# nkkk98/MyGPURaytracer

Measured on AMD Instinct MI355X. Metric: Mrays/s, higher is better.
Workload: dtype f32; 1 GPU; cornellObj.txt 1920x1080 depth 8, AA on, material sort on, 1 spp/step (BASELINE configs[3] / C4); arith=0, clock_warmup_steps=1188, rccl_ranks=1, parallelism=1 GPU

## Files before the change

mygpuraytracer_amd/csrc/pt_engine.hip:

```cpp
#include <hip/hip_runtime.h>
#include <stdint.h>
#include <stdio.h>
#include <string.h>
#include <string>
#include <vector>
#include <algorithm>
#include <cmath>

#include "../../include/mi355x_pathtracer.h"
#include "pt_kernels.h"
#include "pt_scene.h"
#include "pt_denoise.h"

namespace {

thread_local std::string g_last_error;
int set_error(int code, const std::string &msg) { g_last_error = msg; return code; }

#define HIPCHECK(expr)                                                                                   \
    do {                                                                                                 \
        hipError_t e_ = (expr);                                                                          \
        if (e_ != hipSuccess)                                                                            \
            return set_error(PTX_ERR_HIP, std::string(#expr) + ": " + hipGetErrorString(e_));            \
    } while (0)
// ... 205 lines not shown
    hipEvent_t ev_start = nullptr, ev_stop = nullptr;
    bool timing_valid = false;
    ptx_options opt{};
    DCamera cam{};
    int traceDepth = 0;
    TileMap tm{};
    int nbins = 1, nmats = 0, ngeoms = 0, maxTiles = 0, grid = 0, grid_seg = 0, cap = 0, cus = 0;
    bool grid_forced = false;
    int dbg_mesh_wg_per_cu = 0;
    int dbg_extra_lds = 0;
    int dbg_total_wg_per_cu = 0, dbg_nsets = 0;
    DevBuf<DGeom> d_geoms; DevBuf<DMaterial> d_mats; DevBuf<float> d_faces; DevBuf<uint8_t> d_texels;
    float *d_image = nullptr; DevBuf<float> d_image_own;
    DevBuf<float> d_fbuf[3];
    DevBuf<int32_t> d_ibuf[3];
    PathSoA soa[3];
    DevBuf<int32_t> d_counts;
    DevBuf<int32_t> d_chunk;
    DevBuf<int32_t> d_cache_chunk;
    DevBuf<int32_t> d_cache_super;
    int cache_gx = 0;
    DevBuf<int32_t> d_totals;
    int32_t *d_super = nullptr;
    DevBuf<float> d_tri9, d_gtab, d_aabb, d_objcull;
    std::vector<float> h_aabb;
    std::vector<int32_t> h_geom_type, h_roots, h_depths, h_wroots, h_wneeds;
    DevBuf<uint32_t> d_tile_geoms; bool tile_geoms_valid = false;
    DevBuf<BvhQuad> d_bvh_nodes; DevBuf<float> d_bvh_tris; DevBuf<int32_t> d_bvh_root, d_bvh_depth;
    DevBuf<BvhWide4> d_bvh_wide; DevBuf<int32_t> d_bvh_wroot, d_bvh_wneed;
    DevBuf<float> d_fnorm, d_cnorm;
    DevBuf<float> d_ldsblob;
    bool no_fast = false;
    bool no_last = false;
    bool force_fast = false;
    DevBuf<unsigned long long> d_keys; DevBuf<uint32_t> d_items; DevBuf<int32_t> d_item_count;
    DevBuf<int32_t> d_tile_done;
    size_t seg_items = 0;
    int nsuper = 1;
    size_t totals_bytes = 0, seg_totals = 0, field_stride = 0, seg_part = 0;
    int kmax = 1;
    long long split_min_paths = 1LL << 20;
    int lanes = 1;
    hipStream_t lane_stream[MAX_LANES] = {};
    hipEvent_t ev_fork = nullptr, ev_join[MAX_LANES] = {}, ev_chain[MAX_LANES] = {};
    struct Ahead { int first = 0, count = 0, next = 0, unfolded = 0; bool use_cache = false, valid = false, timed = false;
                   unsigned long long dir_bins = ~0ull, ntab_bins = 0ull; };
    Ahead ahead[MAX_LANES];
    int ahead_cur = -1, ahead_nxt = -1;
    bool render_ahead = false;
    int last_ahead_lane = -1;
    hipEvent_t ev_ahead0[MAX_LANES] = {}, ev_ahead1[MAX_LANES] = {};
    bool aux_dirty[MAX_LANES] = {};
    unsigned long long cache_dir_bins = ~0ull, cache_ntab_bins = 0ull;
    int cache_idx16 = 0;
    DevBuf<uchar4> d_pbo;
    DevBuf<float> d_denoised;
    DevBuf<float> d_albedo;
    DevBuf<float4> d_gbuf, d_dn_tmp;
    DevBuf<float> d_dn_out;
    bool gbuf_valid = false, dn_done = false;
    std::vector<uint8_t> h_spec;
    DevBuf<uint8_t> d_spec;
    DevBuf<float> d_var;
    bool var_done = false;
    DevBuf<unsigned long long> d_stamps;
    DevBuf<float> d_part;
// ... 146 lines not shown
    const int nb = t->nbins;
    const int ntri_lds = t->split_mesh ? 0 : t->ntri_lds;
    const int triWords = t->tri_lds ? sceneTableWords(ntri_lds, t->nmats, t->ngeoms) : 0;
    const size_t lds_bounce = sizeof(int32_t) * (bounceLdsWords(triWords, nb) + (t->split_mesh ? QUEUE_WORDS : 0)) + (size_t)t->dbg_extra_lds;
    const bool cache_on = t->cache_active();
    const bool use_cache = cache_on && t->cache_valid && iter_first != 1;
    const bool fill_cache = cache_on && !use_cache;
    const bool batched = K > 1 || t->lanes > 1;
    const bool needs_albedo = t->d_albedo && iter_first == 1;
    const bool fast_unsplit = !t->split_mesh && !t->no_fast && batched && !t->uses_uv && t->opt.sort_by_material &&
                              !needs_albedo && t->cull == 1 && t->tri_lds && t->bump_bits == 0 && t->ntri_lds == t->ntri &&
                              !t->d_bvh_root;
    auto per_cu = [&](bool first_bounce, bool last_bounce = false) {
        if (fast_unsplit && !defer && last_bounce) { if (const char *e = getenv("PTX_DEBUG_WG_LAST")) return std::max(1, atoi(e)); }
        if (fast_unsplit && !defer) { if (const char *e = getenv(first_bounce ? "PTX_DEBUG_WG_FIRST" : "PTX_DEBUG_WG_LATER")) return std::max(1, atoi(e)); }
        if (fast_unsplit) return defer ? PT_FAST_WAVES - 2 : first_bounce ? 20 : PT_FAST_WAVES;
        return t->split_mesh ? 32 : 8;
    };
    auto gx_of = [&](bool first_bounce, bool last_bounce = false) {
        int grid = t->grid_forced ? t->grid : t->cus * per_cu(first_bounce, last_bounce);
        if (t->dbg_total_wg_per_cu > 0) grid = t->cus * t->dbg_total_wg_per_cu;
        int g = grid / K;
        if (!t->grid_forced && t->dbg_total_wg_per_cu <= 0) {
            const int base = t->cus * (fast_unsplit ? (defer ? PT_FAST_WAVES - 2 : PT_FAST_WAVES) : t->split_mesh ? 16 : 8) / K;
            g = std::min(g, std::max(base, t->maxTiles / 8));
        }
        if (g < 64 && t->dbg_total_wg_per_cu <= 0) g = 64;
        if (g > t->maxTiles) g = t->maxTiles;
        if (g > t->grid_seg) g = t->grid_seg;
        if (g > grid) g = grid;
        return g < 1 ? 1 : g;
    };
    const int gx_first = gx_of(true), gx_later = gx_of(false);
    const int gx_last = gx_of(false, true);
    const int grid = t->cus * (t->dbg_total_wg_per_cu > 0 ? t->dbg_total_wg_per_cu : per_cu(false));
    const int gx = gx_later;
    const int nsuper = (gx + 63) / 64;
    const size_t chunk_cap = (size_t)nb * t->grid_seg;
    const size_t seg_counts = (2 * (size_t)nb + 1) * t->maxTiles, seg_chunk = 2 * 3 * chunk_cap, seg_totals = t->seg_totals;
    int32_t *counts_all = t->d_counts + seg0 * seg_counts, *counts_scat = counts_all + (size_t)nb * t->maxTiles;
    auto chunks = [&](int bounce) { return t->d_chunk + seg0 * seg_chunk + (size_t)(bounce & 1) * 3 * chunk_cap; };
    auto totals = [&](int bounce, int which) { return t->d_totals + seg0 * seg_totals + ((size_t)bounce * 2 + which) * nb; };
    auto supers = [&](int bounce, int which) { return t->d_super + seg0 * seg_totals + ((size_t)bounce * 2 + which) * nb * t->nsuper; };
    if (t->aux_dirty[lane]) {
        HIPCHECK(hipMemsetAsync(t->d_totals + seg0 * seg_totals, 0, sizeof(int32_t) * seg_totals * (size_t)t->kmax, stream));
        if (t->d_part)
            HIPCHECK(hipMemset2DAsync(t->d_part + seg0 * t->seg_part + 3 * (size_t)t->cap, sizeof(float) * t->seg_part, 0,
                                      (size_t)t->cap / 8, (size_t)t->kmax, stream));
        t->aux_dirty[lane] = false;
    }

    auto kt_begin = [&](int kind) -> int {
        if (!t->ktiming) return PTX_OK;
        if (t->kev_used + 2 > t->kev.size()) {
            hipEvent_t a, b2;
            HIPCHECK(hipEventCreate(&a)); HIPCHECK(hipEventCreate(&b2));
            t->kev.push_back(a); t->kev.push_back(b2);
        }
        if (t->kev_kind.size() < t->kev.size() / 2) t->kev_kind.resize(t->kev.size() / 2);
        t->kev_kind[t->kev_used / 2] = kind;
        HIPCHECK(hipEventRecord(t->kev[t->kev_used], stream));
        return PTX_OK;
    };
    auto kt_end = [&]() -> int {
        if (!t->ktiming) return PTX_OK;
        HIPCHECK(hipEventRecord(t->kev[t->kev_used + 1], stream));
        t->kev_used += 2;
// ... 22 lines not shown
        for (int k = 0; k < 3; k++) if (bp.sc.cull && !(std::fabs(t->cam.position[k]) <= 0.5f * CULL_FAR_ORIGIN)) bp.sc.cull = 2;
        bp.sc.ldsblob = t->d_ldsblob;
        const bool from_cache = (b == 1 && cache_on), to_cache = (first && cache_on);
        bp.in = from_cache ? t->soa[2] : soa_shift(t->soa[b & 1], seg0 * t->cap);
        bp.stage = to_cache ? t->soa[2] : soa_shift(t->soa[1 - (b & 1)], seg0 * t->cap);
        bp.in_totals = first ? nullptr : from_cache ? t->d_cache_totals : totals(b - 1, 0);
        bp.in_super = first ? nullptr : from_cache ? t->d_cache_super : supers(b - 1, 0);
        bp.in_chunk = first ? nullptr : from_cache ? t->d_cache_chunk : chunks(b - 1);
        const int gx_b = first ? gx_first : gx_later;
        bp.in_gx = from_cache ? t->cache_gx : (b == 1 ? gx_first : gx_later);
        bp.seg_in_totals = from_cache ? 0 : seg_totals; bp.seg_in_chunk = from_cache ? 0 : seg_chunk;
        bp.image = t->d_image;
        bp.iter = iter_first; bp.iter_stride = stride; bp.traceDepth = t->traceDepth; bp.bounce = b;
        bp.aa = t->opt.antialiasing; bp.dof = t->opt.depth_of_field; bp.sort = t->opt.sort_by_material; bp.uses_uv = t->uses_uv; bp.dir_bins = batch_dir_bins;
        bp.ntab_bins = batch_ntab_bins; bp.apps = t->opt.apps_variant; bp.albedo = t->d_albedo;
        bp.in_dir_bins = from_cache ? t->cache_dir_bins : bp.dir_bins; bp.in_ntab_bins = from_cache ? t->cache_ntab_bins : bp.ntab_bins;
        auto idx16_of = [&](int gxw) { return (!getenv("PTX_DEBUG_NO_IDX16") && (t->maxTiles + gxw - 1) / std::max(gxw, 1) <= 128) ? 1 : 0; };
        bp.idx16 = idx16_of(first ? gx_first : gx_later);
        bp.in_idx16 = first ? 0 : from_cache ? t->cache_idx16 : idx16_of(b == 1 ? gx_first : gx_later);
        bp.nbins = nb; bp.maxTiles = t->maxTiles;
        bp.counts_all = counts_all; bp.counts_scat = counts_scat;
        bp.chunk = to_cache ? t->d_cache_chunk : chunks(b); bp.chunk_cap = (int32_t)chunk_cap;
        bp.super_all = supers(b, 0); bp.super_scat = supers(b, 1);
        bp.totals_all = totals(b, 0); bp.totals_scat = totals(b, 1);
        bp.nsuper = t->nsuper;
        bp.seg_in = from_cache ? 0 : (size_t)t->cap; bp.seg_stage = to_cache ? 0 : (size_t)t->cap;
        bp.seg_counts = seg_counts; bp.seg_chunk = to_cache ? 0 : seg_chunk; bp.seg_totals = seg_totals;
        bp.stamps = t->d_stamps;
        bp.seg_part = t->seg_part;
        bp.part = batched ? t->d_part + seg0 * bp.seg_part : nullptr;
        bp.emit_count = (first && fill_cache) ? t->d_emit_count : nullptr;
        bp.emit_pix = t->d_emit_pix; bp.emit_rgb = t->d_emit_rgb;
        bp.fenced = reinterpret_cast<unsigned long long *>(t->d_stats + 65); bp.fence_slots = t->fence_slots; bp.fence_slots_cap = (uint32_t)t->cap;
        bp.tile_geoms = (first && t->tile_geoms_valid) ? t->d_tile_geoms : nullptr;
        if (t->split_mesh) {
            bp.keys = t->d_keys + seg0 * (size_t)t->cap; bp.seg_keys = (size_t)t->cap;
            bp.items = t->d_items + seg0 * t->seg_items; bp.seg_items = t->seg_items;
            bp.item_count = t->d_item_count + 2 * seg0;
            bp.item_cursor = bp.item_count + K;
            bp.tile_done = (first && t->d_tile_done) ? t->d_tile_done + seg0 * (size_t)t->maxTiles : nullptr;
            HIPCHECK(hipMemsetAsync(bp.item_count, 0, sizeof(int32_t) * 2 * (size_t)K, stream));
            KT(first ? 0 : 1, { int rcl = launch_bounce(t, first, 1, needs_albedo, dim3(gx_b, K), lds_bounce, stream, bp); if (rcl != PTX_OK) return rcl; });
            const int mesh_gx = std::max(1, t->cus * (t->dbg_mesh_wg_per_cu > 0 ? t->dbg_mesh_wg_per_cu : PT_MESH_WG_PER_CU) / K);
            KT(2, { t->ks->mesh(first ? 1 : 0, dim3(mesh_gx, K), sizeof(int32_t) * ((size_t)t->bvh_stack * 256 + 32 * MESH_GEOM_WORDS), stream, &bp, t->bvh_stack);
                    t->ks->finish(first ? 1 : 0, dim3(std::max(1, grid / K), K), stream, &bp); });
            const size_t lds_pass2 = sizeof(int32_t) * ((size_t)ldsHeadWords(nb) + TILE);
            KT(3, { int rcl = launch_bounce(t, first, 2, needs_albedo, dim3(gx_b, K), lds_pass2, stream, bp); if (rcl != PTX_OK) return rcl; });
        } else {
            bp.keys = nullptr; bp.items = nullptr; bp.item_count = nullptr; bp.item_cursor = nullptr; bp.seg_keys = bp.seg_items = 0; bp.tile_done = nullptr;
            KT(first ? 0 : 1, { int rcl = launch_bounce(t, first, 0, needs_albedo, dim3(gx_b, K), lds_bounce, stream, bp, gx_last); if (rcl != PTX_OK) return rcl; });
        }

        if (first && fill_cache) {
            HIPCHECK(hipMemcpyAsync(t->d_cache_totals, totals(0, 0), sizeof(int32_t) * 2 * nb, hipMemcpyDeviceToDevice, stream));
            HIPCHECK(hipMemcpyAsync(t->d_cache_super, supers(0, 0), sizeof(int32_t) * 2 * nb * t->nsuper, hipMemcpyDeviceToDevice, stream));
            t->cache_gx = gx_b;
            t->cache_dir_bins = bp.dir_bins; t->cache_ntab_bins = bp.ntab_bins; t->cache_idx16 = bp.idx16;
            t->cache_valid = true;
        }
        if (t->capture_bounce == b && t->d_cap && b + 1 < t->traceDepth) {
            int32_t *gs = t->d_cap + 3 * (size_t)t->cap + nb, *ga = gs + chunk_cap + 1;
            hipLaunchKernelGGL(k_capture_prefix, dim3(1), dim3(64), 0, stream, bp.chunk, (int)chunk_cap, nb * gx_b, gs, ga);
            hipLaunchKernelGGL(k_capture, dim3(std::min(1024, (t->cap + 255) / 256)), dim3(256), 0, stream, bp.stage, bp.chunk, (int)chunk_cap,
                               nb * gx_b, gs, ga, t->cap, t->d_cap, t->d_cap_f, bp.idx16);
            HIPCHECK(hipMemcpyAsync(t->d_cap + 3 * (size_t)t->cap, totals(b, 1), sizeof(int32_t) * nb, hipMemcpyDeviceToDevice, stream));
            t->cap_filled = true;
// ... 189 lines not shown
    t->tm.tile_rows = opt.tile_world > 1 ? opt.tile_rows : H;
    fastdiv_magic((uint32_t)W, t->tm.w_mul, t->tm.w_sh);
    fastdiv_magic((uint32_t)t->tm.tile_rows, t->tm.rows_mul, t->tm.rows_sh);
    t->tm.owned = owned_pixels(W, H, t->tm.tile_rows, opt.tile_rank, opt.tile_world);
    t->maxTiles = (std::max(t->tm.owned, 1) + TILE - 1) / TILE;
    t->cap = t->maxTiles * TILE;
    t->nbins = opt.sort_by_material ? (nmaterials > 0 ? nmaterials : 1) : 1;
    {
        int per_cu = 16;
        if (const char *e = getenv("PTX_DEBUG_WG_PER_CU")) { per_cu = std::max(1, atoi(e)); t->grid_forced = true; }
        t->cus = prop.multiProcessorCount;
        t->grid = std::max(1, std::min(t->maxTiles, prop.multiProcessorCount * per_cu));
    }
    t->grid_seg = std::max(1, std::min(t->grid, t->maxTiles));
    t->nsuper = (t->grid_seg + 63) / 64;
    HostScene hs;
    SceneSwitches sw;
    sw.no_wide_bvh = getenv("PTX_DEBUG_NO_WIDE_BVH") != nullptr; sw.no_chunks = getenv("PTX_DEBUG_NO_CHUNKS") != nullptr;
    sw.no_dir_skip = getenv("PTX_DEBUG_NO_DIR_SKIP") != nullptr; sw.no_normal_codes = getenv("PTX_DEBUG_NO_NORMAL_CODES") != nullptr;
    sw.force_split = getenv("PTX_DEBUG_FORCE_SPLIT") != nullptr; sw.no_objcull = getenv("PTX_DEBUG_NO_OBJCULL") != nullptr;
    if (const int rc = pt_prepare_scene(ngeoms, geoms, nmaterials, materials, opt, t->tm.owned, t->nbins, prop.sharedMemPerBlock, sw, hs)) return fail(rc);
    static_cast<SceneFacts &>(*t) = hs;
    {
        size_t mem_free = 0, mem_total = 0;
        if (opt.batch <= 0 && hipMemGetInfo(&mem_free, &mem_total) != hipSuccess) { mem_free = mem_total = 0; (void)hipGetLastError(); }
        const char *e = getenv("PTX_DEBUG_MEM_BUDGET_MB");
        const LaunchPlan plan = plan_launch_sets(t->tm.owned, t->nbins, t->maxTiles, opt, kmax_cap, mem_free, mem_total, e ? std::max(1LL, atoll(e)) : 0);
        if (!plan.refusal.empty()) { set_error(PTX_ERR_UNSUPPORTED, plan.refusal); return fail(PTX_ERR_UNSUPPORTED); }
        t->kmax = *kmax_used = plan.kmax;
        t->lanes = plan.lanes;
    }
    t->no_fast = getenv("PTX_DEBUG_NO_FAST") != nullptr;
    t->no_last = getenv("PTX_DEBUG_NO_LAST") != nullptr;
    t->force_fast = getenv("PTX_DEBUG_FORCE_FAST") != nullptr;
    if (const char *e = getenv("PTX_DEBUG_TOTAL_WG_PER_CU")) t->dbg_total_wg_per_cu = std::max(0, atoi(e));
    if (const char *e = getenv("PTX_DEBUG_NSETS")) t->dbg_nsets = std::max(0, atoi(e));
    if (const char *e = getenv("PTX_DEBUG_EXTRA_LDS")) t->dbg_extra_lds = std::max(0, std::min(atoi(e), 32768)) & ~15;
    if (const char *e = getenv("PTX_DEBUG_MESH_WG_PER_CU")) t->dbg_mesh_wg_per_cu = std::max(0, atoi(e));
    if (const char *e = getenv("PTX_DEBUG_SPLIT_MIN")) t->split_min_paths = std::max(1LL, atoll(e));
    if (stream) { t->stream = (hipStream_t)stream; t->own_stream = false; }
    else {
        int prio_lo = 0, prio_hi = 0;
        if (hipDeviceGetStreamPriorityRange(&prio_lo, &prio_hi) != hipSuccess) { prio_lo = prio_hi = 0; (void)hipGetLastError(); }
        if (getenv("PTX_DEBUG_NO_PRIORITY")) prio_hi = prio_lo;
        HC(hipStreamCreateWithPriority(&t->stream, hipStreamNonBlocking, prio_hi));
        t->own_stream = true;
    }
    HC(hipEventCreate(&t->ev_start)); HC(hipEventCreate(&t->ev_stop));
    if (t->lanes > 1) {
        HC(hipEventCreateWithFlags(&t->ev_fork, hipEventDisableTiming));
        for (int l = 0; l < t->lanes; l++) {
            if (l) {
                int prio_lo = 0, prio = 0;
                if (hipDeviceGetStreamPriorityRange(&prio_lo, &prio) != hipSuccess || getenv("PTX_DEBUG_NO_PRIORITY")) { prio = 0; (void)hipGetLastError(); }
                if (const char *e = getenv("PTX_DEBUG_LANE_PRIO")) {
                    const char *q = e;
                    for (int k = 1; k <= l && q; k++) { prio = atoi(q); q = strchr(q, ','); if (q) q++; }
                }
                HC(hipStreamCreateWithPriority(&t->lane_stream[l], hipStreamNonBlocking, prio));
            }
            HC(hipEventCreateWithFlags(&t->ev_join[l], hipEventDisableTiming));
            HC(hipEventCreateWithFlags(&t->ev_chain[l], hipEventDisableTiming));
            if (l) { HC(hipEventCreate(&t->ev_ahead0[l])); HC(hipEventCreate(&t->ev_ahead1[l])); }
        }
    }
    HC(t->d_geoms.upload(hs.geoms)); HC(t->d_mats.upload(hs.mats)); HC(t->d_faces.upload(hs.faces)); HC(t->d_texels.upload(hs.texels));
// ... 861 lines not shown
```

mygpuraytracer_amd/csrc/pt_kernels.h:

```cpp
#pragma once
#include <hip/hip_runtime.h>
#include <stdint.h>

#include "pt_device.h"
#include "pt_bvh.h"

using namespace ptd;

namespace {

#ifndef PT_TILE
#define PT_TILE 256
#endif
#ifndef PT_MESH_WAVES
#define PT_MESH_WAVES 5
#endif
#ifndef PT_PARK_STATE
#define PT_PARK_STATE 1
#endif
#ifndef PT_FAST_WAVES
#define PT_FAST_WAVES 8
#endif
#ifndef PT_FAST_WAVES_FIRST
#define PT_FAST_WAVES_FIRST (PT_FAST_WAVES - 1)
#endif
#ifndef PT_FAST_WAVES_SPLIT
#define PT_FAST_WAVES_SPLIT 4
#endif
#ifndef PT_FAST_WAVES_SPLIT2
#define PT_FAST_WAVES_SPLIT2 5
#endif
#ifndef PT_BOUNCE_WAVES
#define PT_BOUNCE_WAVES 4
#endif
constexpr int TILE = PT_TILE;
constexpr int WAVES = TILE / 64;
constexpr int RANK_BITS = TILE <= 256 ? 8 : 9, BIN_BITS = 32 - 2 * RANK_BITS;
static_assert(TILE <= 512 && (TILE & (TILE - 1)) == 0, "tile size: a power of two up to 512 (9-bit ranks)");
#ifndef PT_WIN
#define PT_WIN 32
#endif
constexpr int WIN = PT_WIN, WIN_WORDS = 2 * (WIN + 1) + WIN + 2;
constexpr int ldsHeadWords(int nb) { return ((2 * WAVES * nb + 4 * nb + 1 + 8 + WIN_WORDS) + 3) & ~3; }
constexpr int REC_WORDS = 17 * TILE;
#ifndef PT_REC_ROWS_FAST0
#define PT_REC_ROWS_FAST0 16
#endif
constexpr int REC_ROWS_FAST0 = PT_REC_ROWS_FAST0;
static_assert(WIN <= 64 && (WIN & (WIN - 1)) == 0, "window of runs: one wave, binary search");
__host__ __device__ constexpr size_t bounceLdsWords(int tableWords, int nb) { return (size_t)tableWords + (size_t)ldsHeadWords(nb) + REC_WORDS; }
static_assert(ldsHeadWords(1) % 4 == 0 && ldsHeadWords(2) % 4 == 0 && ldsHeadWords(3) % 4 == 0 && ldsHeadWords(7) % 4 == 0 &&
// ... 102 lines not shown
struct TileMap {
    int32_t W, H, tile_rows, tile_rank, tile_world, owned;
    uint32_t w_mul, w_sh, rows_mul, rows_sh;
};

__device__ __forceinline__ int fastdiv(int n, uint32_t mul, uint32_t sh) {
    return sh == 255u ? n : (int)(__umulhi((uint32_t)n, mul) >> sh);
}

__device__ __forceinline__ void owned_pixel(const TileMap &tm, int i, int &x, int &y) {
    int r = fastdiv(i, tm.w_mul, tm.w_sh);
    x = i - r * tm.W;
    if (tm.tile_world <= 1) { y = r; return; }
    int k = fastdiv(r, tm.rows_mul, tm.rows_sh);
    y = (k * tm.tile_world + tm.tile_rank) * tm.tile_rows + (r - k * tm.tile_rows);
}

__device__ __forceinline__ int slot_to_pixel(const TileMap &tm, int slot) {
    if (tm.tile_world <= 1) return slot;
    int x, y;
    owned_pixel(tm, slot, x, y);
    return x + y * tm.W;
}

struct BounceParams {
    DScene sc;
    DCamera cam;
    TileMap tm;
    PathSoA in, stage;
    const int32_t *in_totals;
    const int32_t *in_super;
    const int32_t *in_chunk;
    int32_t in_gx;
    size_t seg_in_totals, seg_in_chunk;
    float *image;
    int32_t iter, traceDepth, bounce;
    int32_t iter_stride;
    unsigned long long *keys; uint32_t *items; int32_t *item_count;
    int32_t *item_cursor;
    size_t seg_keys, seg_items;
    const uint32_t *tile_geoms;
    int32_t *tile_done;
    int32_t aa, dof, sort;
    int32_t uses_uv;
    unsigned long long dir_bins;
    unsigned long long in_dir_bins, in_ntab_bins;
    int32_t idx16, in_idx16;
    unsigned long long ntab_bins;
    int32_t apps;
    float *albedo;
    int32_t nbins, maxTiles;
    int32_t *counts_all, *counts_scat;
    int32_t *chunk;
    int32_t chunk_cap;
    int32_t *super_all, *super_scat;
    int32_t *totals_all, *totals_scat;
    int32_t nsuper;
    size_t seg_in, seg_stage, seg_counts, seg_chunk, seg_totals, seg_part;
    unsigned long long *stamps;
    float *part;
    int32_t *emit_count; int32_t *emit_pix; float *emit_rgb;
    unsigned long long *fenced;
    uint32_t fence_slots;
    uint32_t fence_slots_cap;
};

// ... 79 lines not shown
```

mygpuraytracer_amd/csrc/pt_kernels.hip:

```cpp
#if PT_ARITH == 1
#define ptd ptd_arith1
#elif PT_ARITH == 2
#define ptd ptd_arith2
#elif defined(PT_ARITH) && PT_ARITH != 0
#error "PT_ARITH must be 0, 1 or 2"
#endif
#include <string.h>

#include "pt_kernels.h"

namespace {

__device__ __forceinline__ int32_t stage_key(int bin, int r_all, int r_scat) { return (int32_t)((uint32_t)bin | ((uint32_t)r_all << BIN_BITS) | ((uint32_t)r_scat << (BIN_BITS + RANK_BITS))); }
__device__ __forceinline__ void fence_report(const BounceParams &p) { atomicAdd(p.fenced, 1ull); }

__device__ __forceinline__ int sum_totals(const int32_t *t, int n) {
    int s = 0;
    for (int b = 0; b < n; b++) s += t[b];
    return s;
}

constexpr int ITEMS_PER_PASS = 4;
#ifdef PT_STAMPS
#define TI_STAMP(k) do { unsigned long long t1_ = __builtin_amdgcn_s_memtime(); st_acc[k] += t1_ - st_t0; st_t0 = t1_; } while (0)
#define TI_ARGS , unsigned long long *st_acc, unsigned long long &st_t0
#define TI_PASS , st_acc, st_t0
#else
#define TI_STAMP(k) do { } while (0)
#define TI_ARGS
#define TI_PASS
#endif
template <bool DEFER, bool PARK = false, bool SUBSET = false, bool DECODE = true>
__device__ __forceinline__ void tileIntersect(const DScene &sc, bool alive, Ray ray, bool need_uv, Hit &hit, int32_t *scratch,
                                              int32_t *tcnt, int &q, int tid, int lane, int wave, unsigned long long &key_out,
                                              uint32_t &mesh_out TI_ARGS, uint32_t subset = 0xffffffffu) {
    const float *gtab = reinterpret_cast<const float *>(pt_lds) + sc.ntri_lds * 24 + sc.nmats * 11;
    float *rayb = reinterpret_cast<float *>(scratch);
    unsigned long long *best = reinterpret_cast<unsigned long long *>(scratch + 6 * TILE);
    uint16_t *list = reinterpret_cast<uint16_t *>(scratch + 8 * TILE);
    uint16_t *listM = list + ITEMS_PER_PASS * TILE;
    constexpr int CAP = ITEMS_PER_PASS * TILE;
    uint32_t cube_mask = 0, sph_mask = 0, mesh_mask = 0;
    if (alive) {
        const uint32_t m = cullMask<SUBSET>(sc, ray, subset);
        cube_mask = m & sc.cube_bits; sph_mask = m & sc.sphere_bits; mesh_mask = m & sc.mesh_bits;
    }
    mesh_out = mesh_mask;
    if (DEFER) mesh_mask = 0;
    rayb[0 * TILE + tid] = ray.o.x; rayb[1 * TILE + tid] = ray.o.y; rayb[2 * TILE + tid] = ray.o.z;
    rayb[3 * TILE + tid] = ray.d.x; rayb[4 * TILE + tid] = ray.d.y; rayb[5 * TILE + tid] = ray.d.z;
    best[tid] = KEY_NONE;
    for (;;) {
        const int cc = (int)__popc(cube_mask), cs = (int)__popc(sph_mask), cm = (int)__popc(mesh_mask);
        const int nc = cc < ITEMS_PER_PASS ? cc : ITEMS_PER_PASS;
        const int ns = cs < ITEMS_PER_PASS - nc ? cs : ITEMS_PER_PASS - nc;
        const int nm = cm < ITEMS_PER_PASS - nc - ns ? cm : ITEMS_PER_PASS - nc - ns;
        int base[3], tot[3];
        const int cnt3[3] = {nc, ns, nm};
#pragma unroll
        for (int kind = 0; kind < 3; kind++) {
            const unsigned long long b0 = __ballot(cnt3[kind] & 1), b1 = __ballot(cnt3[kind] & 2), b2 = __ballot(cnt3[kind] & 4);
            base[kind] = wavePrefix(b0, lane) + 2 * wavePrefix(b1, lane) + 4 * wavePrefix(b2, lane);
            tot[kind] = __popcll(b0) + 2 * __popcll(b1) + 4 * __popcll(b2);
        }
        const unsigned long long left = __ballot(cc + cs + cm > nc + ns + nm);
        int wb0 = 0, wb1 = 0, wb2 = 0;
        if (lane == 0) {
            if (tot[0]) wb0 = atomicAdd(&tcnt[4 * q + 0], tot[0]);
            if (tot[1]) wb1 = atomicAdd(&tcnt[4 * q + 1], tot[1]);
            if (tot[2]) wb2 = atomicAdd(&tcnt[4 * q + 2], tot[2]);
            if (left) tcnt[4 * q + 3] = 1;
        }
        base[0] += __builtin_amdgcn_readfirstlane(wb0);
        base[1] += __builtin_amdgcn_readfirstlane(wb1);
        base[2] += __builtin_amdgcn_readfirstlane(wb2);
        for (int j = 0; j < nc; j++) {
            const int g = __ffs((int)cube_mask) - 1;
            cube_mask &= cube_mask - 1;
            list[base[0] + j] = (uint16_t)(tid | (g << RANK_BITS));
        }
        for (int j = 0; j < ns; j++) {
            const int g = __ffs((int)sph_mask) - 1;
            sph_mask &= sph_mask - 1;
            list[CAP - 1 - (base[1] + j)] = (uint16_t)(tid | (g << RANK_BITS));
        }
        for (int j = 0; j < nm; j++) {
            const int g = __ffs((int)mesh_mask) - 1;
            mesh_mask &= mesh_mask - 1;
            listM[base[2] + j] = (uint16_t)(tid | (g << RANK_BITS));
        }
        __syncthreads();
        const int totC = tcnt[4 * q + 0], totS = tcnt[4 * q + 1], totM = tcnt[4 * q + 2], more = tcnt[4 * q + 3];
        if (tid < 4) tcnt[4 * (q ^ 1) + tid] = 0;
        TI_STAMP(5);
#ifdef PT_STAMPS
        if (tid == 0) { st_acc[8] += totC + totS; st_acc[9] += totM; st_acc[10] += 1; }
#endif
        const int startS = (totC + 63) & ~63, startM = startS + ((totS + 63) & ~63);
// ... 147 lines not shown
template <bool FIRST, int MODE_, bool FAST = false>
__global__ __launch_bounds__(TILE, !FAST ? PT_BOUNCE_WAVES : MODE_ == 1 ? PT_FAST_WAVES_SPLIT : MODE_ == 2 ? PT_FAST_WAVES_SPLIT2 : FIRST ? PT_FAST_WAVES_FIRST : PT_FAST_WAVES) void k_bounce(const BounceParams p_in) {
    constexpr bool LAST = MODE_ == MODE_LAST;
    constexpr int MODE = LAST ? 0 : MODE_;
    static_assert(MODE_ >= 0 && MODE_ <= MODE_LAST && !(LAST && FIRST), "modes 0-2, and the light-only variant of a later unsplit bounce");
#ifdef PT_WGCLOCK
    const unsigned long long wg_t0 = wall_clock64();
#endif
    BounceParams p = p_in;
    if (FAST && MODE != 0) {
        p.sort = 1; p.albedo = nullptr; p.emit_count = nullptr; p.sc.cull = 1; p.sc.tri_lds = 1;
    }
    if (FAST && MODE == 0) {
        p.uses_uv = 0; p.sort = 1; p.albedo = nullptr; p.emit_count = nullptr; p.dof = 0;
        p.sc.cull = 1; p.sc.tri_lds = 2; p.sc.bump_bits = 0; p.sc.ntri_lds = p.sc.ntri; p.sc.bvh_root = nullptr;
    }
    const int tid = threadIdx.x, lane = tid & 63, wave = tid >> 6;
    const int nb = p.nbins;
    const int triWords = (MODE != 2 && p.sc.tri_lds) ? sceneLdsWords(p.sc) : 0;
    int32_t *lds = pt_lds + triWords;
    int32_t *w_all = lds, *w_scat = lds + WAVES * nb;
    int32_t *run_all = lds + 2 * WAVES * nb, *run_scat = run_all + nb;
    int32_t *tcs = run_scat + nb, *toff = tcs + nb;
    int32_t *tcnt = toff + nb + 1;
    int32_t *win = tcnt + 8;
    int tq = 0;
    int32_t *rec = lds + ldsHeadWords(nb);
    constexpr int R_PIX = (FAST && MODE == 0 ? REC_ROWS_FAST0 : 17) - 3, R_MG = R_PIX + 1, R_KEY = R_PIX + 2;
    uint32_t *qbuf = reinterpret_cast<uint32_t *>(rec + REC_WORDS);
    int32_t *qcnt = rec + REC_WORDS + QCAP, *qbase = qcnt + 1;
    if (MODE == 1 && tid == 0) *qcnt = 0;
    for (int k = tid; k < 2 * nb; k += TILE) run_all[k] = 0;
    if (tid < 8) tcnt[tid] = 0;
    __syncthreads();
    const int seg = blockIdx.y;
    const int iter = p.iter + seg * p.iter_stride;
    const PathSoA in_k = soa_offset(p.in, p.seg_in * seg), stage_k = soa_offset(p.stage, p.seg_stage * seg);
    int32_t *counts_all = p.counts_all + p.seg_counts * seg, *counts_scat = p.counts_scat + p.seg_counts * seg;
    int32_t *tile_np = counts_all + 2 * (size_t)nb * p.maxTiles;
    const bool direct = PT_DIRECT_STORE && MODE != 2 && (FAST || nb <= 64);
    int32_t *chunk_out = p.chunk + p.seg_chunk * seg;
    int32_t *super_all = p.super_all + p.seg_totals * seg, *super_scat = p.super_scat + p.seg_totals * seg;
    int32_t *totals_all = p.totals_all + p.seg_totals * seg, *totals_scat = p.totals_scat + p.seg_totals * seg;
    float *part = (FAST || p.part) ? p.part + p.seg_part * seg : nullptr;
    const bool batched = FAST || part != nullptr;
    const int32_t *in_totals = FIRST ? nullptr : p.in_totals + p.seg_in_totals * seg;
    const int32_t *in_chunk = FIRST ? nullptr : p.in_chunk + p.seg_in_chunk * seg;
    const int in_nruns = nb * p.in_gx;
    int v_tot = 0;
    if (!FIRST && nb <= 64 && lane < nb) v_tot = in_totals[nb + lane];
    const int n_in = FIRST ? p.tm.owned : nb <= 64 ? __builtin_amdgcn_readlane(waveInclusiveScan(v_tot, lane), 63) : sum_totals(in_totals + nb, nb);
    const int ntiles = (n_in + TILE - 1) / TILE;
    const int chunk = (ntiles + (int)gridDim.x - 1) / (int)gridDim.x;
    const int tile0 = min((int)blockIdx.x * chunk, ntiles), tile1 = min(tile0 + chunk, ntiles);
    auto binRanges = [&](unsigned long long mask, int &lo0, int &len0, int &lo1, int &len1) {
        int lo[2] = {0, 0}, hi[2] = {0, 0}, nr = 0, pos = 0;
        bool open = false;
        for (int b = 0; b < nb; b++) {
            const int tot = __builtin_amdgcn_readlane(v_tot, b);
            if (tot > 0) {
                const bool set = (mask >> b) & 1ull;
                if (set && !open) { if (nr < 2) lo[nr] = pos; open = true; }
                else if (!set && open) { if (nr < 2) hi[nr] = pos; nr++; open = false; }
            }
            pos += tot;
        }
// ... 76 lines not shown
    };
    auto fetch = [&](uint32_t li4, int idx_base, InRec &r, int jp) -> bool {
        const PathSoA in = soa_fresh(in_k);
        const uint32_t w = (uint32_t)ld_u(in.lsrc(), li4);
        uint32_t j;
        if (p.in_idx16) { j = (li4 >> 2) + (uint32_t)(int32_t)(int16_t)(w & 0xffffu); r.idx = idx_base + (int)(w >> 16); }
        else { j = w; r.idx = idx_base + ld_u(in.lidx(), li4); }
        if (__builtin_expect(j >= p.fence_slots, 0)) fence_report(p);
        const uint32_t j4 = min(j, p.fence_slots - 1u) << 2;
        const bool with_dir = (uint32_t)(jp - dir_lo0) < (uint32_t)dir_len0 || (uint32_t)(jp - dir_lo1) < (uint32_t)dir_len1;
        const bool coded_n = (uint32_t)(jp - ntab_lo0) < (uint32_t)ntab_len0 || (uint32_t)(jp - ntab_lo1) < (uint32_t)ntab_len1;
        typedef float quad __attribute__((ext_vector_type(4)));
        const uint32_t j16 = j4 << 2;
        const quad A = ld_u(reinterpret_cast<const quad *>(in.quadA()), j16), B = ld_u(reinterpret_cast<const quad *>(in.quadB()), j16);
        r.f[0] = A.x; r.f[1] = A.y; r.f[2] = A.z; r.pix = __float_as_int(A.w);
        r.f[6] = B.x; r.f[7] = B.y; r.f[8] = B.z; r.mg = __float_as_int(B.w);
        r.f[3] = r.f[4] = r.f[5] = 0.f; r.f[9] = r.f[10] = r.f[11] = 0.f; r.f[12] = r.f[13] = 0.f;
        if (with_dir) { const quad D = ld_u(reinterpret_cast<const quad *>(in.quadD()), j16); r.f[3] = D.x; r.f[4] = D.y; r.f[5] = D.z; if (p.uses_uv) r.f[13] = D.w; }
        if (!coded_n) { const quad C = ld_u(reinterpret_cast<const quad *>(in.quadC()), j16); r.f[9] = C.x; r.f[10] = C.y; r.f[11] = C.z; if (p.uses_uv) r.f[12] = C.w; }
        if (coded_n) {
            const int g = (int)min((uint32_t)(r.mg >> 16), (uint32_t)(p.sc.ngeoms - 1));
            const vec3 n = cubeNormalByCode(p.sc, reinterpret_cast<const float *>(pt_lds) + p.sc.ntri_lds * 24 + p.sc.nmats * 11, g, (r.pix >> 28) & 7);
            r.f[9] = n.x; r.f[10] = n.y; r.f[11] = n.z;
            r.pix &= 0x0fffffff;
        }
        if (__builtin_expect((uint32_t)r.pix >= (uint32_t)p.tm.owned, 0)) { fence_report(p); r.pix = 0; return false; }
        return true;
    };
    auto classifyRay = [&](const Hit &hit, const PathState &ps, int pix, int &bin, bool &pending) {
        classifyPath<FIRST>(p, iter, part, batched, hit, ps.color, pix, bin, pending);
    };
    int32_t *ccnt = qcnt + 2;
    int n_last = 0;
    int32_t k1_next = 0;
    if (MODE == 2) {
        for (int k = tid; k < 2 * WAVES * nb; k += TILE) lds[k] = 0;
        __syncthreads();
    }
    if (MODE == 2 && !FIRST && tile0 < tile1 && tile0 * TILE + tid < n_in) k1_next = ld_u(soa_fresh(stage_k).lsrc(), (uint32_t)(tile0 * TILE + tid) << 2);
    for (int tile = tile0; tile < tile1; tile++) {
#ifdef PT_STAMPS
        st_t0 = __builtin_amdgcn_s_memtime();
#endif
        const int i = tile * TILE + tid;
        bool alive = i < n_in;
        uint32_t tile_subset = 0xffffffffu;
        if (FIRST && MODE != 2 && p.tile_geoms) tile_subset = ((const __attribute__((address_space(4))) uint32_t *)p.tile_geoms)[tile];
        InRec cur;
        uint32_t li4 = 0;
        int idx_base = 0;
        if (!FIRST && MODE != 2) locate(tile, li4, idx_base);
        const PathSoA stage = soa_fresh(stage_k);
        PathState ps;
        int pix = 0;
        if (MODE != 2 && !direct && !LAST) for (int k = tid; k < 2 * WAVES * nb; k += TILE) lds[k] = 0;
        ps.o = ps.d = ps.color = V3(0.f, 0.f, 0.f);
        unsigned long long key = KEY_NONE;
        int32_t k1 = 0;
        if (MODE == 2 && !FIRST) {
            k1 = k1_next;
            if (tile + 1 < tile1 && i + TILE < n_in) k1_next = ld_u(soa_fresh(stage_k).lsrc(), (uint32_t)(i + TILE) << 2);
        }
        if (MODE == 2 && FIRST && p.tile_done && (p.tile_done + (size_t)p.maxTiles * seg)[tile]) {
            for (int b = tid; b < nb; b += TILE) {
                const int ca = counts_all[(size_t)b * p.maxTiles + tile], cs = counts_scat[(size_t)b * p.maxTiles + tile];
                counts_all[(size_t)b * p.maxTiles + tile] = run_all[b];
// ... 21 lines not shown
                owned_pixel(p.tm, i, x, y);
                pix = i;
                if (tile_subset != 0u) generateRay(p.cam, iter, p.traceDepth, p.aa != 0, p.dof != 0, x, y, ps);
            } else {
                const bool rec_ok = fetch(li4, idx_base, cur, min(i, n_in - 1));
                const vec3 intersect = V3(cur.f[0], cur.f[1], cur.f[2]);
                ps.d = V3(cur.f[3], cur.f[4], cur.f[5]);
                ps.color = V3(cur.f[6], cur.f[7], cur.f[8]);
                pix = cur.pix;
                Hit h;
                h.t = 1.f;
                h.n = V3(cur.f[9], cur.f[10], cur.f[11]);
                h.u = cur.f[12]; h.v = cur.f[13];
                const int mg = cur.mg;
                h.mat = mg & 0xffff; h.geom = mg >> 16;
                const int sidx = cur.idx;
#ifdef PT_STAMPS
                asm volatile("s_waitcnt vmcnt(0)" ::: "memory");
                STAMP(11);
#endif
                Rng rng; rng.seed(iter, sidx, 0);
                bool ended = (FAST && MODE == 0) ? scatterRay<false>(p.sc, ps, intersect, h, getMaterial(p.sc, h.mat), rng)
                                                 : scatterRay<true>(p.sc, ps, intersect, h, getMaterial(p.sc, h.mat), rng);
                if (ended && rec_ok) deposit(p.tm, p.image, part, batched, pix, ps.color, p.apps, p.fence_slots_cap);
                if (ended || !rec_ok) alive = false;
            }
        }
        STAMP(0);
        if (LAST) {
            n_last += __popcll(__ballot(alive));
            if (p.sc.light_bits == 0u) continue;
            Ray ray; ray.o = ps.o; ray.d = ps.d;
            const bool reach = alive && cullMask<true>(p.sc, ray, p.sc.light_bits) != 0u;
            Hit none;
            uint32_t mesh_cand = 0;
            tileIntersect<false, false, false, false>(p.sc, reach, ray, false, none, rec, tcnt, tq, tid, lane, wave, key, mesh_cand TI_PASS);
            if (reach && key != KEY_NONE) {
                const float *G = reinterpret_cast<const float *>(pt_lds) + p.sc.ntri_lds * 24 + p.sc.nmats * 11 + (int)((key >> 24) & 0xff) * GTAB_WORDS;
                Hit lh;
                lh.t = 1.f; lh.n = V3(0.f, 0.f, 0.f); lh.u = lh.v = 0.f; lh.geom = 0; lh.ncode = 0;
                lh.mat = __float_as_int(G[37]);
                int lbin = 0;
                bool lpend = false;
                classifyRay(lh, ps, pix, lbin, lpend);
            }
            STAMP(1);
            continue;
        }
        Hit hit;
        hit.t = -1.f; hit.n = V3(0.f, 0.f, 0.f); hit.u = hit.v = 0.f; hit.geom = 0; hit.mat = 0; hit.ncode = 0;
        if (FIRST && MODE == 0 && tile_subset == 0u) {
            int mbin = 0;
            bool mpend = false;
            if (alive) classifyRay(hit, ps, pix, mbin, mpend);
            if (tid == 0) tile_np[tile] = 0;
            if (tid == 0) run_all[p.sort ? p.sc.nmats - 1 : 0] += min(TILE, n_in - tile * TILE);
            continue;
        }
        if (FIRST && MODE == 1 && tile_subset == 0u && p.tile_done) {
            int mbin = 0;
            bool mpend = false;
            if (alive) classifyRay(hit, ps, pix, mbin, mpend);
            if (tid == 0) tile_np[tile] = 0;
            const int missbin = p.sort ? p.sc.nmats - 1 : 0, nalive = min(TILE, n_in - tile * TILE);
            for (int b = tid; b < nb; b += TILE) {
                counts_all[(size_t)b * p.maxTiles + tile] = b == missbin ? nalive : 0;
                counts_scat[(size_t)b * p.maxTiles + tile] = 0;
            }
            if (tid == 0) (p.tile_done + (size_t)p.maxTiles * seg)[tile] = 1;
            continue;
        }
        {
            Ray ray; ray.o = ps.o; ray.d = ps.d;
            uint32_t mesh_cand = 0;
            if (MODE == 1) {
                if (FIRST && tile_subset == 0u) __syncthreads();
                else tileIntersect<true, false, FIRST>(p.sc, alive, ray, p.uses_uv != 0, hit, rec, tcnt, tq, tid, lane, wave, key, mesh_cand TI_PASS, tile_subset);
// ... 58 lines not shown
            else {
                if (alive) intersectScene(p.sc, ray, hit);
                __syncthreads();
            }
        }
        STAMP(1);
    classify:
        if (MODE != 2 && direct && lane < nb) { w_all[wave * nb + lane] = 0; w_scat[wave * nb + lane] = 0; }
        if (MODE != 2 && alive) classifyRay(hit, ps, pix, bin, pending);
        STAMP(2);
        int r_all = 0, r_scat = 0;
        {
            const int abin = alive ? bin : -1, pbin = pending ? bin : -1;
            if (PT_RANK_SLICED && MODE != 2 && !FIRST && nb <= 16) {
                const unsigned long long A = __builtin_amdgcn_uicmp((uint32_t)abin, 0xffffffffu, 33), P = __builtin_amdgcn_uicmp((uint32_t)pbin, 0xffffffffu, 33);
                uint32_t slo = 0xffffffffu, shi = 0xffffffffu;
#pragma unroll
                for (int k = 0; k < 4; k++) {
                    if (k && (nb - 1) >> k == 0) break;
                    const unsigned long long Bk = __builtin_amdgcn_uicmp((uint32_t)bin & (1u << k), 0u, 33);
                    const bool set = (bin >> k) & 1;
                    slo &= set ? (uint32_t)Bk : ~(uint32_t)Bk;
                    shi &= set ? (uint32_t)(Bk >> 32) : ~(uint32_t)(Bk >> 32);
                }
                const uint32_t alo = slo & (uint32_t)A, ahi = shi & (uint32_t)(A >> 32), plo = slo & (uint32_t)P, phi = shi & (uint32_t)(P >> 32);
                const int ra = (int)__builtin_amdgcn_mbcnt_hi(ahi, __builtin_amdgcn_mbcnt_lo(alo, 0u));
                const int rs = (int)__builtin_amdgcn_mbcnt_hi(phi, __builtin_amdgcn_mbcnt_lo(plo, 0u));
                if (alive) {
                    r_all = ra; r_scat = rs;
                    if (ra == 0) {
                        w_all[wave * nb + bin] = __popc(alo) + __popc(ahi);
                        w_scat[wave * nb + bin] = __popc(plo) + __popc(phi);
                    }
                }
            } else {
                unsigned long long remaining = __builtin_amdgcn_uicmp((uint32_t)abin, 0xffffffffu, 33);
                while (remaining) {
                    int leader = __ffsll((long long)remaining) - 1;
                    int b = __builtin_amdgcn_readlane(abin, leader);
                    const unsigned long long m_all = __builtin_amdgcn_uicmp((uint32_t)abin, (uint32_t)b, 32), m_scat = __builtin_amdgcn_uicmp((uint32_t)pbin, (uint32_t)b, 32);
                    const int ra = wavePrefix(m_all, lane), rs = wavePrefix(m_scat, lane);
                    if (abin == b) { r_all = ra; r_scat = rs; }
                    if (lane == leader) {
                        w_all[wave * nb + b] = __popcll(m_all);
                        w_scat[wave * nb + b] = __popcll(m_scat);
                    }
                    remaining &= ~m_all;
                }
            }
        }
        STAMP(12);
        __syncthreads();
        STAMP(13);
        if (alive) {
            for (int w = 0; w < wave; w++) { r_all += w_all[w * nb + bin]; r_scat += w_scat[w * nb + bin]; }
        }
        int toff_bin = 0, npend_r = 0;
        if (direct) {
            int ln = lane;
            asm volatile("" : "+v"(ln));
            int ca = 0, cs = 0;
            if (ln < nb) for (int w = 0; w < WAVES; w++) { ca += w_all[w * nb + ln]; cs += w_scat[w * nb + ln]; }
            if (wave == 0 && ln < nb) {
                counts_all[(size_t)ln * p.maxTiles + tile] = MODE == 1 ? ca : run_all[ln];
                counts_scat[(size_t)ln * p.maxTiles + tile] = MODE == 1 ? cs : run_scat[ln];
                run_all[ln] += ca;
// ... 619 lines not shown
```

Before: 43140 Mrays/s.

## Compact last-bounce light rays into LDS pool and add wave-uniform fast paths

In the last-bounce light-reach pass, rays that can reach a light are compacted into a shared LDS pool across tiles and intersected only once a full tile's worth has accumulated. This cuts the number of idle lanes during light intersection. The change also adds a wave-uniform fast path for slot allocation in tileIntersect and for binning in the classify step. The packed-scan slot allocation replaces the three-ballot prefix computation. These changes add extra syncthreads and reuse the rec scratch buffer for the pool, which risks LDS aliasing with tileIntersect's own use of that scratch.

```diff
diff --git a/mygpuraytracer_amd/csrc/pt_engine.hip b/mygpuraytracer_amd/csrc/pt_engine.hip
--- a/mygpuraytracer_amd/csrc/pt_engine.hip
+++ b/mygpuraytracer_amd/csrc/pt_engine.hip
@@ -261,6 +261,7 @@
     DevBuf<float> d_ldsblob;
     bool no_fast = false;
     bool no_last = false;
+    bool last_inplace = false;
     bool force_fast = false;
     DevBuf<unsigned long long> d_keys; DevBuf<uint32_t> d_items; DevBuf<int32_t> d_item_count;
     DevBuf<int32_t> d_tile_done;
@@ -473,7 +474,8 @@
         return g < 1 ? 1 : g;
     };
     const int gx_first = gx_of(true), gx_later = gx_of(false);
-    const int gx_last = gx_of(false, true);
+    int gx_last = gx_of(false, true);
+    if (const char *e = getenv("PTX_DEBUG_GX_LAST")) gx_last = std::max(1, std::min(atoi(e), gx_last));
     const int grid = t->cus * (t->dbg_total_wg_per_cu > 0 ? t->dbg_total_wg_per_cu : per_cu(false));
     const int gx = gx_later;
     const int nsuper = (gx + 63) / 64;
@@ -562,6 +564,7 @@
         bp.emit_count = (first && fill_cache) ? t->d_emit_count : nullptr;
         bp.emit_pix = t->d_emit_pix; bp.emit_rgb = t->d_emit_rgb;
         bp.fenced = reinterpret_cast<unsigned long long *>(t->d_stats + 65); bp.fence_slots = t->fence_slots; bp.fence_slots_cap = (uint32_t)t->cap;
+        bp.last_inplace = t->last_inplace ? 1 : 0;
         bp.tile_geoms = (first && t->tile_geoms_valid) ? t->d_tile_geoms : nullptr;
         if (t->split_mesh) {
             bp.keys = t->d_keys + seg0 * (size_t)t->cap; bp.seg_keys = (size_t)t->cap;
@@ -817,6 +820,7 @@
     }
     t->no_fast = getenv("PTX_DEBUG_NO_FAST") != nullptr;
     t->no_last = getenv("PTX_DEBUG_NO_LAST") != nullptr;
+    t->last_inplace = getenv("PTX_DEBUG_LAST_INPLACE") != nullptr;
     t->force_fast = getenv("PTX_DEBUG_FORCE_FAST") != nullptr;
     if (const char *e = getenv("PTX_DEBUG_TOTAL_WG_PER_CU")) t->dbg_total_wg_per_cu = std::max(0, atoi(e));
     if (const char *e = getenv("PTX_DEBUG_NSETS")) t->dbg_nsets = std::max(0, atoi(e));
diff --git a/mygpuraytracer_amd/csrc/pt_kernels.h b/mygpuraytracer_amd/csrc/pt_kernels.h
--- a/mygpuraytracer_amd/csrc/pt_kernels.h
+++ b/mygpuraytracer_amd/csrc/pt_kernels.h
@@ -17,6 +17,12 @@
 #endif
 #ifndef PT_PARK_STATE
 #define PT_PARK_STATE 1
+#endif
+#ifndef PT_PACKED_SLOTS
+#define PT_PACKED_SLOTS 1
+#endif
+#ifndef PT_WAVE_UNIFORM
+#define PT_WAVE_UNIFORM 1
 #endif
 #ifndef PT_FAST_WAVES
 #define PT_FAST_WAVES 8
@@ -185,6 +191,7 @@
     const int32_t *in_super;
     const int32_t *in_chunk;
     int32_t in_gx;
+    int32_t last_inplace;
     size_t seg_in_totals, seg_in_chunk;
     float *image;
     int32_t iter, traceDepth, bounce;
diff --git a/mygpuraytracer_amd/csrc/pt_kernels.hip b/mygpuraytracer_amd/csrc/pt_kernels.hip
--- a/mygpuraytracer_amd/csrc/pt_kernels.hip
+++ b/mygpuraytracer_amd/csrc/pt_kernels.hip
@@ -30,6 +30,7 @@
 #define TI_ARGS
 #define TI_PASS
 #endif
+__device__ __forceinline__ int waveInclusiveScan(int v, int lane);
 template <bool DEFER, bool PARK = false, bool SUBSET = false, bool DECODE = true>
 __device__ __forceinline__ void tileIntersect(const DScene &sc, bool alive, Ray ray, bool need_uv, Hit &hit, int32_t *scratch,
                                               int32_t *tcnt, int &q, int tid, int lane, int wave, unsigned long long &key_out,
@@ -40,13 +41,18 @@
     uint16_t *list = reinterpret_cast<uint16_t *>(scratch + 8 * TILE);
     uint16_t *listM = list + ITEMS_PER_PASS * TILE;
     constexpr int CAP = ITEMS_PER_PASS * TILE;
-    uint32_t cube_mask = 0, sph_mask = 0, mesh_mask = 0;
+    uint32_t cube_mask = 0, sph_mask = 0, mesh_mask = 0, m_all = 0;
     if (alive) {
-        const uint32_t m = cullMask<SUBSET>(sc, ray, subset);
-        cube_mask = m & sc.cube_bits; sph_mask = m & sc.sphere_bits; mesh_mask = m & sc.mesh_bits;
+        m_all = cullMask<SUBSET>(sc, ray, subset);
+        cube_mask = m_all & sc.cube_bits; sph_mask = m_all & sc.sphere_bits; mesh_mask = m_all & sc.mesh_bits;
     }
     mesh_out = mesh_mask;
     if (DEFER) mesh_mask = 0;
+    bool uniform_wave = false;
+    if (SUBSET && PT_WAVE_UNIFORM) {
+        const uint32_t m0 = (uint32_t)__builtin_amdgcn_readfirstlane((int)m_all);
+        uniform_wave = __ballot(alive && m_all == m0) == ~0ull && __popc(m0 & (DEFER ? ~sc.mesh_bits : 0xffffffffu)) <= ITEMS_PER_PASS;
+    }
     rayb[0 * TILE + tid] = ray.o.x; rayb[1 * TILE + tid] = ray.o.y; rayb[2 * TILE + tid] = ray.o.z;
     rayb[3 * TILE + tid] = ray.d.x; rayb[4 * TILE + tid] = ray.d.y; rayb[5 * TILE + tid] = ray.d.z;
     best[tid] = KEY_NONE;
@@ -56,14 +62,29 @@
         const int ns = cs < ITEMS_PER_PASS - nc ? cs : ITEMS_PER_PASS - nc;
         const int nm = cm < ITEMS_PER_PASS - nc - ns ? cm : ITEMS_PER_PASS - nc - ns;
         int base[3], tot[3];
-        const int cnt3[3] = {nc, ns, nm};
+        unsigned long long left = 0ull;
+        if (SUBSET && PT_WAVE_UNIFORM && uniform_wave) {
+            const int u0 = __builtin_amdgcn_readfirstlane(nc), u1 = __builtin_amdgcn_readfirstlane(ns), u2 = __builtin_amdgcn_readfirstlane(nm);
+            base[0] = lane * u0; base[1] = lane * u1; base[2] = lane * u2;
+            tot[0] = 64 * u0; tot[1] = 64 * u1; tot[2] = 64 * u2;
+        } else {
+#if PT_PACKED_SLOTS
+            const int packed = nc | (ns << 10) | (nm << 20);
+            const int inc = waveInclusiveScan(packed, lane), exc = inc - packed;
+            const int all = __builtin_amdgcn_readlane(inc, 63);
+            base[0] = exc & 1023; base[1] = (exc >> 10) & 1023; base[2] = exc >> 20;
+            tot[0] = all & 1023; tot[1] = (all >> 10) & 1023; tot[2] = all >> 20;
+#else
+            const int cnt3[3] = {nc, ns, nm};
 #pragma unroll
-        for (int kind = 0; kind < 3; kind++) {
-            const unsigned long long b0 = __ballot(cnt3[kind] & 1), b1 = __ballot(cnt3[kind] & 2), b2 = __ballot(cnt3[kind] & 4);
-            base[kind] = wavePrefix(b0, lane) + 2 * wavePrefix(b1, lane) + 4 * wavePrefix(b2, lane);
-            tot[kind] = __popcll(b0) + 2 * __popcll(b1) + 4 * __popcll(b2);
-        }
-        const unsigned long long left = __ballot(cc + cs + cm > nc + ns + nm);
+            for (int kind = 0; kind < 3; kind++) {
+                const unsigned long long b0 = __ballot(cnt3[kind] & 1), b1 = __ballot(cnt3[kind] & 2), b2 = __ballot(cnt3[kind] & 4);
+                base[kind] = wavePrefix(b0, lane) + 2 * wavePrefix(b1, lane) + 4 * wavePrefix(b2, lane);
+                tot[kind] = __popcll(b0) + 2 * __popcll(b1) + 4 * __popcll(b2);
+            }
+#endif
+            left = __ballot(cc + cs + cm > nc + ns + nm);
+        }
         int wb0 = 0, wb1 = 0, wb2 = 0;
         if (lane == 0) {
             if (tot[0]) wb0 = atomicAdd(&tcnt[4 * q + 0], tot[0]);
@@ -277,6 +298,7 @@
     if (MODE == 1 && tid == 0) *qcnt = 0;
     for (int k = tid; k < 2 * nb; k += TILE) run_all[k] = 0;
     if (tid < 8) tcnt[tid] = 0;
+    if (LAST && tid == 0) tcs[0] = 0;
     __syncthreads();
     const int seg = blockIdx.y;
     const int iter = p.iter + seg * p.iter_stride;
@@ -419,6 +441,7 @@
     };
     int32_t *ccnt = qcnt + 2;
     int n_last = 0;
+    int32_t *pool_n = tcs;
     int32_t k1_next = 0;
     if (MODE == 2) {
         for (int k = tid; k < 2 * WAVES * nb; k += TILE) lds[k] = 0;
@@ -506,17 +529,51 @@
             if (p.sc.light_bits == 0u) continue;
             Ray ray; ray.o = ps.o; ray.d = ps.d;
             const bool reach = alive && cullMask<true>(p.sc, ray, p.sc.light_bits) != 0u;
-            Hit none;
-            uint32_t mesh_cand = 0;
-            tileIntersect<false, false, false, false>(p.sc, reach, ray, false, none, rec, tcnt, tq, tid, lane, wave, key, mesh_cand TI_PASS);
-            if (reach && key != KEY_NONE) {
-                const float *G = reinterpret_cast<const float *>(pt_lds) + p.sc.ntri_lds * 24 + p.sc.nmats * 11 + (int)((key >> 24) & 0xff) * GTAB_WORDS;
-                Hit lh;
-                lh.t = 1.f; lh.n = V3(0.f, 0.f, 0.f); lh.u = lh.v = 0.f; lh.geom = 0; lh.ncode = 0;
-                lh.mat = __float_as_int(G[37]);
-                int lbin = 0;
-                bool lpend = false;
-                classifyRay(lh, ps, pix, lbin, lpend);
+            const bool inplace = !FAST || p.last_inplace != 0;
+            const unsigned long long rb = __ballot(reach);
+            int pbase = 0;
+            if (!inplace && lane == 0 && rb) pbase = atomicAdd(pool_n, __popcll(rb));
+            int slot = inplace ? tid : __builtin_amdgcn_readfirstlane(pbase) + wavePrefix(rb, lane);
+            float *poolf = reinterpret_cast<float *>(rec);
+            auto pool_put = [&](int s) {
+                poolf[0 * TILE + s] = ray.o.x; poolf[1 * TILE + s] = ray.o.y; poolf[2 * TILE + s] = ray.o.z;
+                poolf[3 * TILE + s] = ray.d.x; poolf[4 * TILE + s] = ray.d.y; poolf[5 * TILE + s] = ray.d.z;
+                poolf[12 * TILE + s] = ps.color.x; poolf[13 * TILE + s] = ps.color.y; poolf[14 * TILE + s] = ps.color.z;
+                rec[15 * TILE + s] = pix;
+            };
+            if (reach && (uint32_t)slot < (uint32_t)TILE) pool_put(slot);
+            __syncthreads();
+            int total = inplace ? TILE : *pool_n;
+            while (total >= TILE || (tile == tile1 - 1 && total > 0)) {
+                const int n = min(max(total, 0), TILE);
+                const bool pa = tid < n && (!inplace || reach);
+                Ray pr;
+                pr.o = V3(poolf[0 * TILE + tid], poolf[1 * TILE + tid], poolf[2 * TILE + tid]);
+                pr.d = V3(poolf[3 * TILE + tid], poolf[4 * TILE + tid], poolf[5 * TILE + tid]);
+                Hit none;
+                uint32_t mesh_cand = 0;
+                tileIntersect<false, false, false, false>(p.sc, pa, pr, false, none, rec, tcnt, tq, tid, lane, wave, key, mesh_cand TI_PASS);
+                if (tid == 0) *pool_n = total - n;
+                if (pa && key != KEY_NONE) {
+                    const float *G = reinterpret_cast<const float *>(pt_lds) + p.sc.ntri_lds * 24 + p.sc.nmats * 11 + (int)((key >> 24) & 0xff) * GTAB_WORDS;
+                    Hit lh;
+                    lh.t = 1.f; lh.n = V3(0.f, 0.f, 0.f); lh.u = lh.v = 0.f; lh.geom = 0; lh.ncode = 0;
+                    lh.mat = __float_as_int(G[37]);
+                    PathState pps;
+                    pps.o = pr.o; pps.d = pr.d;
+                    pps.color = V3(poolf[12 * TILE + tid], poolf[13 * TILE + tid], poolf[14 * TILE + tid]);
+                    const int ppix = rec[15 * TILE + tid];
+                    int lbin = 0;
+                    bool lpend = false;
+                    if ((uint32_t)ppix < (uint32_t)p.tm.owned) classifyRay(lh, pps, ppix, lbin, lpend);
+                    else fence_report(p);
+                }
+                total -= n;
+                if (!FAST) break;
+                __syncthreads();
+                slot -= TILE;
+                if (reach && (uint32_t)slot < (uint32_t)TILE) pool_put(slot);
+                __syncthreads();
             }
             STAMP(1);
             continue;
@@ -641,6 +698,16 @@
                         w_all[wave * nb + bin] = __popc(alo) + __popc(ahi);
                         w_scat[wave * nb + bin] = __popc(plo) + __popc(phi);
                     }
+                }
+            } else if (PT_WAVE_UNIFORM && FIRST && MODE != 2 && __builtin_amdgcn_uicmp((uint32_t)abin, (uint32_t)__builtin_amdgcn_readfirstlane(abin), 32) == ~0ull &&
+                       __builtin_amdgcn_readfirstlane(abin) >= 0) {
+                const int b = __builtin_amdgcn_readfirstlane(abin);
+                const unsigned long long m_scat = __builtin_amdgcn_uicmp((uint32_t)pbin, (uint32_t)b, 32);
+                r_all = lane;
+                r_scat = m_scat == ~0ull ? lane : m_scat == 0ull ? 0 : wavePrefix(m_scat, lane);
+                if (lane == 0) {
+                    w_all[wave * nb + b] = 64;
+                    w_scat[wave * nb + b] = __popcll(m_scat);
                 }
             } else {
                 unsigned long long remaining = __builtin_amdgcn_uicmp((uint32_t)abin, 0xffffffffu, 33);
```

After: 43970 Mrays/s (median of 6 runs). 1.9% higher.
